# erick093/MPI_Pytorch

Hardware: AMD Instinct MI355X
Metric: images/sec (whole node) ResNet-18 224x224 training at 1/2/4/8 MI355X (higher is better)
Workload: dtype bf16; 1 GPU; model=resnet18, global_batch=2048, per_gpu_batch=2048, image_size=224, num_classes=64500, optimizer=adam, parallelism=dp1, device=cuda, backend=none, hip_graph=False, deterministic=True

## Files before the change

### csrc/bindings.cpp

```cpp
#include <torch/extension.h>
#include <c10/hip/HIPStream.h>
#include <c10/core/DeviceGuard.h>

#include <vector>

#include "kernels/api.h"
#include "runtime/runtime.h"

using torch::Tensor;

namespace {

inline hipStream_t cur_stream() { return c10::hip::getCurrentHIPStream().stream(); }

#define CHECK_CUDA(x) TORCH_CHECK((x).is_cuda(), #x " must be a GPU tensor")
#define CHECK_CONTIG(x) TORCH_CHECK((x).is_contiguous(), #x " must be contiguous")
#define CHECK_BF16(x) \
  TORCH_CHECK((x).scalar_type() == torch::kBFloat16, #x " must be bfloat16, got ", (x).scalar_type())
#define CHECK_F32(x) \
  TORCH_CHECK((x).scalar_type() == torch::kFloat32, #x " must be float32, got ", (x).scalar_type())
#define CHECK_ACT(x) \
  CHECK_CUDA(x);     \
  CHECK_CONTIG(x);   \
  CHECK_BF16(x)
// ... 425 lines not shown

void bn_defer_step(Tensor sums, Tensor gamma, Tensor mean, Tensor rstd, int64_t s0, Tensor k12,
                   Tensor dgamma, Tensor dbeta, Tensor G, Tensor x, c10::optional<Tensor> out) {
  CHECK_CUDA(G);
  CHECK_CONTIG(G);
  CHECK_ACT(x);
  CHECK_F32(k12);
  CHECK_CONTIG(k12);
  const int Ci = sums.numel() / 2;
  const int ctot = x.size(-1);
  const int M = x.numel() / ctot;
  TORCH_CHECK(x.is_contiguous() && G.sizes() == x.sizes() && k12.numel() == 2 * ctot,
              "bn_defer_step: G / x / k12 shapes");
  TORCH_CHECK(s0 >= 0 && s0 < Ci && Ci <= ctot && (Ci - s0) % 8 == 0 &&
                  256 % ((Ci - s0) / 8) == 0,
              "bn_defer_step: slice [s0, Ci) must be 8-channel groups dividing 256");
  for (const Tensor* t : {&gamma, &mean, &rstd}) {
    CHECK_F32(*t);
    TORCH_CHECK(t->numel() >= Ci, "bn_defer_step: per-channel vector size");
  }
  const bool into = out && out->defined() && out->numel() > 0;
  if (into) {
    CHECK_ACT((*out));
    TORCH_CHECK(out->is_contiguous() && out->size(-1) == Ci - s0 && out->numel() / (Ci - s0) == M,
                "bn_defer_step: out must be a contiguous bf16 [..., Ci - s0]");
  }
  const c10::OptionalDeviceGuard g(device_of(x));
  mpa::bn_defer_step(sums.data_ptr<float>(), gamma.data_ptr<float>(), mean.data_ptr<float>(),
                     rstd.data_ptr<float>(), Ci, (int)s0, M, k12.data_ptr<float>(), ctot,
                     fopt_mut(dgamma), fopt_mut(dbeta), G.data_ptr(),
                     G.scalar_type() == torch::kFloat32, ctot, bp(x), ctot,
                     into ? bpm(*out) : nullptr, cur_stream());
}

static int row_stride(const Tensor& t);

std::vector<Tensor> bn_bwd_apply(Tensor dy, Tensor x, Tensor y, Tensor mean, Tensor rstd,
                                 Tensor gamma, Tensor dgamma, Tensor dbeta, Tensor sums,
                                 bool want_dx, bool want_g) {
  CHECK_CUDA(dy);
  CHECK_BF16(dy);
  const int lddy = row_stride(dy);
  CHECK_ACT(x);
  const int C = x.size(-1);
  const int M = x.numel() / C;
  TORCH_CHECK(C % 8 == 0 && sums.numel() == 2 * C && dy.size(-1) == C && lddy % 8 == 0,
              "bn_bwd_apply: shapes");
  TORCH_CHECK(aligned16(dy),
              "bn_bwd_apply: dy must start on a 16-byte boundary (channel offset % 8 == 0)");
  const c10::OptionalDeviceGuard g(device_of(x));
  Tensor dx = want_dx ? torch::empty_like(x) : Tensor();
  Tensor gout = want_g ? torch::empty_like(x) : Tensor();
  mpa::bn_bwd_apply(bp(dy), bp(x), bopt(y), fopt(mean), fopt(rstd), fopt(gamma),
                    fopt_mut(dgamma), fopt_mut(dbeta), M, C, want_dx ? bpm(dx) : nullptr,
                    want_g ? bpm(gout) : nullptr, fopt(sums), cur_stream(), lddy);
  return {dx, gout};
}

void conv_wgrad(Tensor dy, Tensor x, Tensor dw, int64_t sh, int64_t sw, int64_t ph, int64_t pw,
                bool overwrite) {
  CHECK_ACT(dy);
  CHECK_ACT(x);
  CHECK_CUDA(dw);
  CHECK_F32(dw);
  CHECK_CONTIG(dw);
  const int N = x.size(0), H = x.size(1), W = x.size(2), C = x.size(3);
  const int P = dy.size(1), Q = dy.size(2), K = dy.size(3);
  TORCH_CHECK(dw.dim() == 4 && dw.size(0) == K && dw.size(3) == C, "conv_wgrad: dw shape");
  const int R = dw.size(1), S = dw.size(2);
  TORCH_CHECK(dy.size(0) == N, "conv_wgrad: batch mismatch");
  const c10::OptionalDeviceGuard g(device_of(dy));
  mpa::WGradArgs a{};
  a.dy = bp(dy); a.x = bp(x); a.dw = dw.data_ptr<float>();
  a.Kout = K; a.C = C; a.H = H; a.W = W; a.P = P; a.Q = Q; a.R = R; a.S = S;
  a.sh = sh; a.sw = sw; a.ph = ph; a.pw = pw;
  a.Mpix = N * P * Q;
  a.Ncols = R * S * C;
  a.overwrite = overwrite ? 1 : 0;
  Tensor slab;
  a.slab = alloc_ws(slab, dy, mpa::igemm_wgrad_ws_floats(a.Kout, a.Ncols, a.Mpix));
  mpa::igemm_wgrad(a, vec_width(K), (C % 8 == 0) ? 8 : 1, cur_stream());
}

Tensor act_bwd(Tensor dy, Tensor y, Tensor dbias) {
  CHECK_ACT(dy);
  const int C = dy.size(-1);
  const int M = dy.numel() / C;
  const bool hy = has(y);
  if (!hy && !has(dbias)) return dy;
  const c10::OptionalDeviceGuard g(device_of(dy));
  Tensor out = hy ? torch::empty_like(dy) : dy;
  Tensor ws;
  float* wsp = nullptr;
  if (has(dbias) && C % 8 == 0) {
    ws = torch::empty({mpa::bn_ws_floats(M, C)}, dy.options().dtype(torch::kFloat32));
    wsp = ws.data_ptr<float>();
  }
  mpa::act_bwd(bp(dy), hy ? bopt(y) : nullptr, fopt_mut(dbias), M, C, hy ? bpm(out) : nullptr,
               wsp, cur_stream());
  return out;
}

static uint8_t* ymask_ptr(const c10::optional<Tensor>& m, const Tensor& like) {
  if (!m || !m->defined() || m->numel() == 0) return nullptr;
  TORCH_CHECK(m->scalar_type() == torch::kUInt8 && m->is_contiguous() && m->numel() == like.numel() / 8 &&
                  m->device() == like.device(),
              "bn: ReLU mask must be contiguous uint8 [numel / 8] on the activation's device");
  return m->data_ptr<uint8_t>();
}

static int row_stride(const Tensor& t) {
  TORCH_CHECK(t.dim() >= 1 && t.stride(-1) == 1, "bn: channels must be contiguous");
  if (t.dim() == 1) return (int)t.size(0);
  const int64_t ld = t.stride(-2);
  int64_t expect = ld * t.size(-2);
  for (int64_t d = t.dim() - 3; d >= 0; --d) {
    TORCH_CHECK(t.size(d) == 1 || t.stride(d) == expect, "bn: rows must be uniformly strided");
    expect *= t.size(d);
  }
  TORCH_CHECK(ld >= t.size(-1), "channel window: row stride below the row width");
  return (int)ld;
}

static void bn_prefix(const Tensor& x, int64_t channels, int* C, int* ldx, int* M) {
  CHECK_CUDA(x);
  CHECK_BF16(x);
  if (channels > 0) {
    CHECK_CONTIG(x);
    *ldx = x.size(-1);
    *C = (int)channels;
  } else {
    *ldx = row_stride(x);
    *C = x.size(-1);
  }
  TORCH_CHECK(*C <= *ldx && *C % 8 == 0 && *ldx % 8 == 0,
              "bn: channels must be a multiple of 8 within the row");
  TORCH_CHECK(aligned16(x), "bn: x must start on a 16-byte boundary (channel offset % 8 == 0)");
  *M = x.numel() / x.size(-1);
}

static std::vector<int64_t> with_last(const Tensor& x, int64_t c) {
  std::vector<int64_t> shape(x.sizes().begin(), x.sizes().end());
  shape.back() = c;
  return shape;
}

std::vector<Tensor> bn_fwd_train(Tensor x, Tensor stats, Tensor gamma, Tensor beta, Tensor rmean,
                                 Tensor rvar, double momentum, double eps, Tensor res, bool relu,
                                 c10::optional<Tensor> counter, c10::optional<Tensor> mask,
                                 int64_t channels, c10::optional<Tensor> res_affine,
                                 c10::optional<Tensor> out) {
  int C, ldx, M;
  bn_prefix(x, channels, &C, &ldx, &M);
  const c10::OptionalDeviceGuard g(device_of(x));
  const bool into = out && out->defined() && out->numel() > 0;
  int ldy = C;
  if (into) {
    CHECK_CUDA(*out);
    CHECK_BF16(*out);
    TORCH_CHECK(out->sizes() == c10::IntArrayRef(with_last(x, C)) && !has(res) &&
                    !(mask && mask->defined() && mask->numel()),
                "bn_fwd_train: out must have the output's shape (no residual / mask)");
    ldy = row_stride(*out);
    TORCH_CHECK(ldy % 8 == 0, "bn_fwd_train: out row stride must be a multiple of 8");
    TORCH_CHECK(aligned16(*out),
                "bn_fwd_train: out must start on a 16-byte boundary (channel offset % 8 == 0)");
// ... 1153 lines not shown
  CHECK_CUDA(g);
  CHECK_CONTIG(g);
  CHECK_F32(g);
  const int64_t ctot = g.size(-1);
  TORCH_CHECK(ctot % 8 == 0 && cs % 8 == 0 && off % 8 == 0 && off >= 0 && off + cs <= ctot && cs > 0,
              "chan_extract: channel range outside G (multiples of 8 required)");
  const int64_t pixels = g.numel() / ctot;
  TORCH_CHECK(pixels * (cs / 8) < (int64_t(1) << 31), "chan_extract: too large");
  const c10::OptionalDeviceGuard gd(device_of(g));
  std::vector<int64_t> shape(g.sizes().begin(), g.sizes().end());
  shape.back() = cs;
  Tensor out = torch::empty(shape, g.options().dtype(torch::kBFloat16));
  if (pixels > 0)
    mpa::chan_extract(g.data_ptr<float>(), (int)ctot, (int)off, bpm(out), (int)cs, (int)pixels,
                      cur_stream());
  return out;
}

std::vector<Tensor> split_channels(Tensor dy, std::vector<int64_t> sizes) {
  CHECK_ACT(dy);
  TORCH_CHECK(dy.dim() >= 2 && !sizes.empty(), "split_channels: dy must be [..., C]");
  int64_t ctot = 0;
  for (int64_t c : sizes) {
    TORCH_CHECK(c > 0 && c % 8 == 0, "split_channels: channels must be a multiple of 8");
    ctot += c;
  }
  TORCH_CHECK(ctot == dy.size(-1), "split_channels: sizes do not sum to C");
  const int64_t pixels = dy.numel() / ctot;
  TORCH_CHECK(pixels * (ctot / 8) < (int64_t(1) << 31), "split_channels: too large");
  const c10::OptionalDeviceGuard g(device_of(dy));
  std::vector<Tensor> out;
  std::vector<mpa::bf16_raw*> ptrs;
  std::vector<int> chans;
  std::vector<int64_t> shape(dy.sizes().begin(), dy.sizes().end());
  for (int64_t c : sizes) {
    shape.back() = c;
    out.push_back(torch::empty(shape, dy.options()));
    ptrs.push_back(bpm(out.back()));
    chans.push_back((int)c);
  }
  if (pixels > 0)
    mpa::split_channels(bp(dy), chans.data(), (int)sizes.size(), (int)pixels, (int)ctot,
                        ptrs.data(), cur_stream());
  return out;
}

}

extern "C" const char* mpa_src_hash();

PYBIND11_MODULE(TORCH_EXTENSION_NAME, m) {
  m.doc() = "mpi_pytorch_amd native gfx950 kernels + runtime";
  m.def("src_hash", [] { return std::string(mpa_src_hash()); },
        "hash of the csrc/ sources this binary was built from (setup.py source_hash)");
  m.def("igemm_engine", &mpa::igemm_engine, "GEMM staging engine: 1 LDS-DMA, 0 register");
  m.def("igemm_set_engine", &mpa::igemm_set_engine);
  m.def("igemm_force_tile", &mpa::igemm_force_tile, "override GEMM tile (BM, BN, splits); 0 = auto");
  m.def("igemm_set_tune", &mpa::igemm_set_tune, "tile autotuner on/off (MPA_TUNE)");
  m.def("igemm_set_tune_drain", &mpa::igemm_set_tune_drain,
        "tuner candidates: drain the whole device (1, single GPU) or only their stream (0)");
  m.def("set_deterministic", &mpa::set_deterministic,
        "fixed-order reductions + no timing-based autotuning (MPA_DETERMINISTIC)");
  m.def("deterministic", &mpa::deterministic);
  m.def("igemm_tuned_table", &mpa::igemm_tuned_table, "autotuned GEMM tiles so far");
  m.def("igemm_tuned_load", &mpa::igemm_tuned_load, py::arg("table"), py::arg("replace") = true,
        "adopt an igemm_tuned_table() dump (data-parallel ranks take rank 0's)");
  m.def("igemm_set_dma_uni", &mpa::igemm_set_dma_uni, "LDS-DMA uniform-tap fast path on/off");
  m.def("igemm_set_halo", &mpa::igemm_set_halo, "halo-staged direct 3x3/s1 conv on/off");
  m.def("igemm_set_halo_mi7", &mpa::igemm_set_halo_mi7, "448-pixel halo tiles on/off");
  m.def("igemm_set_halo_strip", &mpa::igemm_set_halo_strip,
        "strip-tiled halo conv: 0 off, 1 images too wide for linear tiles, 2 also layer1");
  m.def("igemm_halo_enabled", &mpa::igemm_halo_enabled);
  m.def("igemm_set_stem", &mpa::igemm_set_stem, "direct row-staged 7x7 pixel-pair stem on/off");
  m.def("preprocess_set_copy", &mpa::preprocess_set_copy,
        "identity-size preprocess fast path on/off (MPA_PRE_COPY)");
  m.def("set_comm_reserve", &mpa::set_comm_reserve,
        "CUs held by an overlapping collective (persistent conv grids use the rest)");
  m.def("comm_reserve", &mpa::comm_reserve, "current collective CU reservation");
  m.def("active_cus", &mpa::active_cus, "CUs the persistent conv grids size for");
  m.def("igemm_set_halo_wprod", &mpa::igemm_set_halo_wprod,
        "halo weight gradients on producer-wave blocks on/off (MPA_HALO_WPROD)");
  m.def("igemm_set_halo_wxmap", &mpa::igemm_set_halo_wxmap,
        "XCD-grouped halo weight-gradient block order on/off (MPA_HALO_WXMAP)");
  m.def("affine_act", &affine_act, "relu?(x * aff[0] + aff[1]) per channel (aff [2, C])");
  m.def("conv_fwd", &conv_fwd, py::arg("x"), py::arg("w"), py::arg("bias"), py::arg("sh"),
        py::arg("sw"), py::arg("ph"), py::arg("pw"), py::arg("relu"), py::arg("stats"),
        py::arg("shift"), "conv forward (+ BN statistics of its output)");
  m.def("conv_dgrad", &conv_dgrad, py::arg("dy"), py::arg("w"), py::arg("H"), py::arg("W"),
        py::arg("sh"), py::arg("sw"), py::arg("ph"), py::arg("pw"), py::arg("wt") = py::none(),
        py::arg("accum") = py::none());
  m.def("conv_wgrad", &conv_wgrad, py::arg("dy"), py::arg("x"), py::arg("dw"), py::arg("sh"),
        py::arg("sw"), py::arg("ph"), py::arg("pw"), py::arg("overwrite") = false,
        "weight gradient into dw (+=; overwrite: dw = ..., the first gradient since zero)");
  m.def("conv_bnred_ok", &conv_bnred_ok);
  m.def("conv_dgrad_bnred_gacc", &conv_dgrad_bnred_gacc);
  m.def("conv_dgrad_res", &conv_dgrad_res);
  m.def("conv_dgrad_pair", &conv_dgrad_pair, py::arg("dy"), py::arg("w"), py::arg("wt"),
        py::arg("H"), py::arg("W"), py::arg("sh"), py::arg("sw"), py::arg("ph"), py::arg("pw"),
        py::arg("dy2"), py::arg("w2"), py::arg("wt2"), py::arg("ph2"), py::arg("pw2"),
        py::arg("accum") = py::none());
  m.def("bn_defer_step", &bn_defer_step, py::arg("sums"), py::arg("gamma"), py::arg("mean"),
        py::arg("rstd"), py::arg("s0"), py::arg("k12"), py::arg("dgamma"), py::arg("dbeta"),
        py::arg("G"), py::arg("x"), py::arg("out") = py::none());
  m.def("conv_fwd_into", &conv_fwd_into);
  m.def("conv_dgrad_bnred", &conv_dgrad_bnred, py::arg("dy"), py::arg("w"), py::arg("H"),
        py::arg("W"), py::arg("sh"), py::arg("sw"), py::arg("ph"), py::arg("pw"), py::arg("wt"),
        py::arg("z"), py::arg("y"), py::arg("mean"), py::arg("rstd"),
        py::arg("gamma") = py::none(), py::arg("beta") = py::none());
  m.def("bn_bwd_apply", &bn_bwd_apply);
  m.def("act_bwd", &act_bwd);
  m.def("bn_fwd_train", &bn_fwd_train, py::arg("x"), py::arg("stats"), py::arg("gamma"),
        py::arg("beta"), py::arg("rmean"), py::arg("rvar"), py::arg("momentum"), py::arg("eps"),
        py::arg("res"), py::arg("relu"), py::arg("counter") = py::none(),
        py::arg("mask") = py::none(), py::arg("channels") = 0,
        py::arg("res_affine") = py::none(), py::arg("out") = py::none());
  m.def("bn_stats_affine", &bn_stats_affine, py::arg("x"), py::arg("stats"), py::arg("gamma"),
        py::arg("beta"), py::arg("rmean"), py::arg("rvar"), py::arg("momentum"),
        py::arg("eps"), py::arg("counter") = py::none());
  m.def("bn_stats", &bn_stats, "[mean | biased var] of x [..., C]");
  m.def("bn_relu_avgpool2_fwd", &bn_relu_avgpool2_fwd);
  m.def("bn_fwd_eval", &bn_fwd_eval, py::arg("x"), py::arg("gamma"), py::arg("beta"),
        py::arg("rmean"), py::arg("rvar"), py::arg("eps"), py::arg("res"), py::arg("relu"),
        py::arg("channels") = 0);
  m.def("bn_bwd_pair", &bn_bwd_pair);
  m.def("maxpool_bwd_relu", &maxpool_bwd_relu);
  m.def("bn_bwd", &bn_bwd, py::arg("dy"), py::arg("x"), py::arg("y"), py::arg("mean"),
        py::arg("rstd"), py::arg("gamma"), py::arg("dgamma"), py::arg("dbeta"),
        py::arg("want_dx"), py::arg("want_g"), py::arg("zmask_beta") = py::none(),
        py::arg("ymask") = py::none(), py::arg("gacc") = py::none(),
        py::arg("dx_out") = py::none());
  m.def("relu_fwd", &relu_fwd);
  m.def("comm_emulator", &comm_emulator, "diagnostics: occupy CUs like a concurrent collective");
  m.def("atomic_latency", &atomic_latency, "diagnostics: dependent atomic round trips");
  m.def("maxpool_fwd", &maxpool_fwd);
  m.def("maxpool_bwd", &maxpool_bwd);
  m.def("bn_relu_maxpool_fwd", &bn_relu_maxpool_fwd, py::arg("z"), py::arg("stats"),
        py::arg("gamma"), py::arg("beta"), py::arg("rmean"), py::arg("rvar"), py::arg("momentum"),
        py::arg("eps"), py::arg("kh"), py::arg("kw"), py::arg("sh"), py::arg("sw"), py::arg("ph"),
        py::arg("pw"), py::arg("ceil"), py::arg("counter") = py::none(),
        py::arg("zsel_out") = py::none());
  m.def("maxpool_bn_bwd_sums", &maxpool_bn_bwd_sums);
  m.def("stem_pool_wgrad_ok", &stem_pool_wgrad_ok);
  m.def("stem_pool_wgrad", &stem_pool_wgrad);
  m.def("maxpool_bn_bwd", &maxpool_bn_bwd, py::arg("dp"), py::arg("idx"), py::arg("z"),
        py::arg("mean"), py::arg("rstd"), py::arg("gamma"), py::arg("beta"), py::arg("dgamma"),
        py::arg("dbeta"), py::arg("kh"), py::arg("kw"), py::arg("sh"), py::arg("sw"),
        py::arg("ph"), py::arg("pw"), py::arg("zsel") = py::none());
  m.def("avgpool_fwd", &avgpool_fwd);
  m.def("avgpool_bwd", &avgpool_bwd, py::arg("dy"), py::arg("H"), py::arg("W"), py::arg("kh"),
        py::arg("kw"), py::arg("sh"), py::arg("sw"), py::arg("ph"), py::arg("pw"),
        py::arg("ceil"), py::arg("cip"), py::arg("dx_out") = py::none());
  m.def("adaptive_avgpool_fwd", &adaptive_avgpool_fwd);
  m.def("adaptive_avgpool_bwd", &adaptive_avgpool_bwd);
  m.def("linear_fwd", &linear_fwd);
  m.def("linear_dgrad", &linear_dgrad, py::arg("dy"), py::arg("w"), py::arg("wt") = py::none());
  m.def("linear_wgrad", &linear_wgrad, py::arg("dy"), py::arg("x"), py::arg("dw"),
        py::arg("overwrite") = false);
  m.def("ce_fwd", &ce_fwd, py::arg("logits"), py::arg("labels"), py::arg("smoothing") = 0.0,
        py::arg("labels2") = py::none(), py::arg("lam") = py::none());
  m.def("ce_bwd", &ce_bwd, py::arg("logits"), py::arg("labels"), py::arg("lse"),
        py::arg("grad_out"), py::arg("weight") = 1.0, py::arg("smoothing") = 0.0,
        py::arg("labels2") = py::none(), py::arg("lam") = py::none());
  m.def("ce_fwd_weighted", &ce_fwd_weighted, py::arg("logits"), py::arg("labels"),
        py::arg("out"), py::arg("acc"), py::arg("weight"), py::arg("accumulate"),
        py::arg("smoothing") = 0.0, py::arg("labels2") = py::none(), py::arg("lam") = py::none());
  m.def("argmax_correct", &argmax_correct);
// ... 43 lines not shown
```

### csrc/kernels/api.h

```cpp
#pragma once
#include <algorithm>
#include <string>
#include <hip/hip_runtime.h>
#include <stdint.h>

namespace mpa {

typedef uint16_t bf16_raw;
constexpr int MAXT = 128;

struct Taps {
  short dh[MAXT];
  short dw[MAXT];
  short bt[MAXT];
};

struct FastDiv {
  uint32_t m, s;
};
inline FastDiv make_fastdiv(uint32_t d) {
  if (d <= 1) return FastDiv{0u, 0u};
  const uint32_t l = 32u - (uint32_t)__builtin_clz(d - 1u);
  return FastDiv{(uint32_t)(((1ull << (31 + l)) + d - 1) / d), l - 1u};
}
// ... 40 lines not shown
  const float* ep_gamma;
  const float* ep_beta;
  void* ep_gacc;
  int ep_gacc_f32;
  int stap;
  int beta;
  FastDiv fd_hw, fd_ow;
  const bf16_raw* A2;
  const bf16_raw* B2;
  int ldb2;
  int kpad;
  const bf16_raw* ep_res;
  const uint8_t* ep_rmask;
};
constexpr short TAP_SRC2 = 0x2000;

inline void igemm_set_fastdiv(IGemmArgs& a) {
  a.fd_hw = make_fastdiv((uint32_t)std::max(1, a.oH * a.oW));
  a.fd_ow = make_fastdiv((uint32_t)std::max(1, a.oW));
  for (int i = 0; i < a.nphase && i < MAXPH; ++i) {
    a.ph[i].fd_hw = make_fastdiv((uint32_t)std::max(1, a.ph[i].oH * a.ph[i].oW));
    a.ph[i].fd_ow = make_fastdiv((uint32_t)std::max(1, a.ph[i].oW));
  }
}

struct WGradArgs {
  const bf16_raw* dy;
  const bf16_raw* x;
  float* dw;
  float* slab;
  int Kout, C, H, W, P, Q, R, S, sh, sw, ph, pw;
  int Mpix;
  int Ncols;
  int ktiles_per_split;
  int tiles_n, tiles_total;
  int overwrite;
};

int64_t igemm_slab_floats(int M, int N);
void igemm_rows(IGemmArgs a, int vw, float* ws, float* slab, hipStream_t s);
void igemm_rows_dgrad(IGemmArgs a, int vw, float* ws, hipStream_t s, bool bkc = false);
void igemm_rows_dgrad_phases(IGemmArgs a, int vw, hipStream_t s, bool bkc = false);
bool igemm_dgrad_src2_ok(const IGemmArgs& a, int vw, bool bkc);
int64_t igemm_bnred_slab_floats(int M, int N, int nphase);
void igemm_rows_dgrad_bnred(IGemmArgs a, int vw, bool bkc, float* slab, float* sums,
                            hipStream_t s);
void igemm_wgrad(WGradArgs a, int vwa, int vwb, hipStream_t s);
int64_t igemm_ws_floats(int M, int N, int Ktot);
int64_t igemm_wgrad_ws_floats(int Kout, int Ncols, int Mpix);
int igemm_engine();
void igemm_set_engine(int engine);
void igemm_force_tile(int bm, int bn, int splits);
void igemm_set_tune(int on);
void igemm_set_tune_drain(int on);
std::string igemm_tuned_table();
int igemm_tuned_load(const std::string& table, bool replace);
void igemm_set_dma_uni(int on);
bool igemm_stap_ok();
bool conv3_halo_ok(const IGemmArgs& a);
int conv3_halo(IGemmArgs a, hipStream_t s);
constexpr int HALO_MAX_ROWS = 256;
void igemm_set_halo(int on);
void igemm_set_halo_mi7(int on);
void igemm_set_halo_strip(int mode);
bool stem_wgrad_ok(const WGradArgs& a);
int stem_wgrad(WGradArgs a, hipStream_t s);
int64_t stem_wgrad_ws_floats();
struct StemPoolArgs {
  const bf16_raw* dp;
  const uint8_t* idx;
  const float *mean, *rstd, *gamma, *beta;
  const float* sums;
  int PP, PQ;
  float invM;
};
bool stem_pool_wgrad_ok(const WGradArgs& a, const StemPoolArgs& q);
int stem_pool_wgrad(WGradArgs a, StemPoolArgs q, hipStream_t s);
void igemm_stem_pool_wgrad(WGradArgs a, StemPoolArgs q, hipStream_t s);
bool conv3_halo_wgrad_ok(const WGradArgs& a);
void igemm_set_halo_wxmap(int on);
void igemm_set_halo_wprod(int on);
int conv3_halo_wgrad(WGradArgs a, hipStream_t s);
int64_t conv3_halo_wgrad_ws_floats(int Kout, int Ncols);
bool igemm_halo_enabled();
void set_comm_reserve(int cus);
int comm_reserve();
int active_cus();
bool conv_stem_ok(const IGemmArgs& a);
int conv_stem(IGemmArgs a, hipStream_t s);
void igemm_set_stem(int on);

int64_t bn_ws_floats(int M, int C);
void slab_reduce(const float* slab, int S, int W, float* out, bool zero_out, hipStream_t s);
bool dense_gacc_ok(const IGemmArgs& a);
void dense_gacc(IGemmArgs a, float* slab, float* sums, hipStream_t s);
void bn_defer_step(const float* sums, const float* gamma, const float* mean, const float* rstd,
                   int Ci, int s0, int M, float* k12, int ldk, float* dgamma, float* dbeta,
                   void* G, bool g_f32, int ldg, const bf16_raw* x, int ldx, bf16_raw* out,
                   hipStream_t s);
void set_deterministic(int on);
bool deterministic();
void slab_stats(float* slab, int S, int C, const float* shift, int M, float* sums, float* out,
                hipStream_t s, int out_ld = 0);
void stats_finalize(const float* sums, const float* shift, int M, int C, float* out,
                    hipStream_t s);
void bn_stats(const bf16_raw* x, int M, int C, const float* shift, float* stats, float* ws,
              hipStream_t s);
void bn_fwd_train(const bf16_raw* x, const float* stats, const float* gamma, const float* beta,
                  float* rmean, float* rvar, float momentum, float eps, const bf16_raw* res,
                  int relu, int M, int C, bf16_raw* y, float* mean, float* rstd,
                  int64_t* counter, hipStream_t s,
                  uint8_t* ymask = nullptr,
                  int ldx = 0,
                  int lds = 0,
                  const float* res_aff = nullptr,
                  int ldy = 0);
void bn_stats_affine(const float* stats, const float* gamma, const float* beta, float* rmean,
                     float* rvar, float momentum, float eps, int M, int C, float* mean,
                     float* rstd, float* aff, int64_t* counter, hipStream_t s);
void bn_relu_avgpool2_fwd(const bf16_raw* z, const float* aff, int N, int H, int W, int C,
                          bf16_raw* y, hipStream_t s);
void affine_act(const bf16_raw* x, const float* aff, int relu, int M, int C, bf16_raw* y,
                hipStream_t s);
void bn_fwd_eval(const bf16_raw* x, const float* gamma, const float* beta, const float* rmean,
                 const float* rvar, float eps, const bf16_raw* res, int relu, int M, int C,
                 bf16_raw* y, hipStream_t s, int ldx = 0);
void bn_bwd(const bf16_raw* dy, const bf16_raw* x, const bf16_raw* y, const float* mean,
            const float* rstd, const float* gamma, float* dgamma, float* dbeta, int M, int C,
            bf16_raw* dx, bf16_raw* g, float* ws, hipStream_t s,
            const float* zmask_beta = nullptr,
            const uint8_t* ymask = nullptr,
            int ldx = 0,
            float* gacc = nullptr,
            int ldg = 0,
            int lddx = 0,
            bool gacc_bf16 = false,
            int lddy = 0);
bool maxpool2_ok(int N, int H, int W, int C, int kh, int kw, int sh, int sw, int ph, int pw);
void maxpool2_fwd(const bf16_raw* x, int N, int H, int W, int C, bf16_raw* y, uint8_t* idx,
                  hipStream_t s);
int64_t maxpool2_ws_floats(int N, int H, int W, int C);
void maxpool2_bwd(const bf16_raw* dy, const uint8_t* idx, const bf16_raw* yp, int N, int H, int W,
                  int C, bf16_raw* dx, float* sums, float* ws, hipStream_t s);
int64_t bn_pair_ws_floats(int M, int C);
void bn_bwd_pair(const bf16_raw* dy, const bf16_raw* x, const bf16_raw* x2, const uint8_t* ymask,
                 const float* mean, const float* rstd, const float* gamma, const float* mean2,
                 const float* rstd2, const float* gamma2, float* dgamma, float* dbeta,
                 float* dgamma2, float* dbeta2, int M, int C, bf16_raw* dx, bf16_raw* dx2,
                 float* ws, hipStream_t s);
void bn_bwd_apply(const bf16_raw* dy, const bf16_raw* x, const bf16_raw* y, const float* mean,
                  const float* rstd, const float* gamma, float* dgamma, float* dbeta, int M,
                  int C, bf16_raw* dx, bf16_raw* g, const float* sums, hipStream_t s,
                  int lddy = 0);
void act_bwd(const bf16_raw* dy, const bf16_raw* y, float* dbias, int M, int C, bf16_raw* g,
             float* ws, hipStream_t s);
void relu_fwd(const bf16_raw* x, int64_t n, bf16_raw* y, hipStream_t s);
void bn_relu_maxpool_fwd(const bf16_raw* z, const float* stats, const float* gamma,
                         const float* beta, float* rmean, float* rvar, float momentum, float eps,
                         int N, int H, int W, int C, int P, int Q, int kh, int kw, int sh, int sw,
                         int ph, int pw, bf16_raw* y, uint8_t* idx, float* mean, float* rstd,
                         int64_t* counter, hipStream_t s, bf16_raw* zsel = nullptr);
int64_t maxpool_bn_ws_floats(int M, int C);
void maxpool_bn_bwd_sums(const bf16_raw* dp, const bf16_raw* zsel, const float* mean,
                         const float* rstd, const float* gamma, const float* beta, float* dgamma,
                         float* dbeta, int MP, int C, float* ws, hipStream_t s);
void maxpool_bn_bwd(const bf16_raw* dp, const uint8_t* idx, const bf16_raw* z, const float* mean,
// ... 140 lines not shown
```

### csrc/kernels/conv_halo.hip

```cpp
#include <algorithm>
#include <atomic>
#include <cstdlib>
#include <type_traits>
#include "igemm_common.h"

namespace mpa {

constexpr int HB_BM = 256, HB_BN = 64, HB_NW = 4;
constexpr int HB_HIW = 9;
constexpr int HB_HPX = 16 * HB_NW * HB_HIW;
constexpr int HB_HBYTES = HB_HPX * 64;
constexpr int HB_WIW = 9;
constexpr int HB_WBYTES = 9 * HB_BN * 64;
constexpr int HB_RED = HB_NW * HB_BN * 2 * 4;
constexpr int HB_COLS = 4 * HB_BN * 4;
constexpr int HB_LDS = 2 * HB_HBYTES + 2 * HB_WBYTES + HB_RED + HB_COLS;

struct HaloPlan {
  int w2;
  int btoff[9];
  uint32_t mag_w, mag_w2, mag_h1, mag_hw;
  int tiles_m, tiles_total, cc;
  uint32_t a_bytes, b_bytes;
};

__device__ __forceinline__ bf16x8 frag16(const char* lds_byte) {
  return __builtin_bit_cast(bf16x8, *LDS_PTR(const u32x4, lds_byte));
}

enum : int { EP_RELU = 1, EP_BETA = 2, EP_BNRED = 4, EP_STATS = 8, EP_BIAS = 16 };

template <int MI = 4>
struct EpiInT {
  uint2 a[MI][4];
  uint2 mk[MI];
};
typedef EpiInT<4> EpiIn;

__device__ __forceinline__ uint2 acc_operand(const IGemmArgs& p, uint32_t e) {
  return *(const uint2*)((const bf16_t*)(p.ep_res ? p.ep_res : p.C) + e);
}

__device__ __forceinline__ uint2 acc_mask(const IGemmArgs& p, uint32_t e0) {
  return p.ep_rmask ? *(const uint2*)(p.ep_rmask + (e0 >> 3)) : make_uint2(~0u, ~0u);
}

__device__ __forceinline__ uint2 masked_acc(uint2 v, uint2 mk, int jn, int jq) {
  const uint32_t word = jn < 2 ? mk.x : mk.y;
  const uint32_t nib = (word >> ((16 * jn + 4 * jq) & 31)) & 15u;
  v.x &= ((nib & 1u) ? 0xffffu : 0u) | ((nib & 2u) ? 0xffff0000u : 0u);
  v.y &= ((nib & 4u) ? 0xffffu : 0u) | ((nib & 8u) ? 0xffff0000u : 0u);
  return v;
}

template <int EPI, int NJ, int MI = 4>
__device__ __forceinline__ void epi_preload(const IGemmArgs& p, EpiInT<MI>& in, int m0, int n0,
                                            int wave, int lane) {
  if constexpr (!(EPI & (EP_BETA | EP_BNRED))) {
#pragma unroll
    for (int i = 0; i < MI; ++i)
#pragma unroll
      for (int jn = 0; jn < 4; ++jn) in.a[i][jn] = make_uint2(0u, 0u);
  } else {
    const int nl = (lane >> 4) * 4;
#pragma unroll
    for (int i = 0; i < MI; ++i) {
      const int m = min(m0 + wave * 16 * MI + i * 16 + (lane & 15), p.M - 1);
      const uint32_t orow = (uint32_t)m * p.ldc + n0 + nl;
      if constexpr (!(EPI & EP_BNRED)) in.mk[i] = acc_mask(p, (uint32_t)m * p.ldc + n0);
#pragma unroll
      for (int jn = 0; jn < NJ; ++jn) {
        if constexpr (EPI & EP_BNRED) {
          in.a[i][jn] = *(const uint2*)(p.ep_z + orow + jn * 16);
        } else {
          in.a[i][jn] = acc_operand(p, orow + jn * 16);
        }
      }
    }
  }
}

__device__ __forceinline__ float lo_f(uint32_t w) { return __uint_as_float(w << 16); }
__device__ __forceinline__ float hi_f(uint32_t w) { return __uint_as_float(w & 0xffff0000u); }

template <int EPI, bool FULL, bool ST = true>
// ... 838 lines not shown
  const int wave_all = __builtin_amdgcn_readfirstlane(tid >> 6);
  const int wave = wave_all & 3;
  const int H = p.H, W = p.W, HW = H * W, W2 = W2T ? W2T : h.w2, C = p.C, K = p.Kout;
  const int M = p.Mpix, nimg = M / HW;
  const int g = lane >> 4, li = lane & 15, q = li >> 2, pp = li & 3;

  const int bid = h.xmap ? (blockIdx.x & 7) * (gridDim.x >> 3) + (blockIdx.x >> 3) : blockIdx.x;
  const int part = bid % h.parts, z = bid / h.parts;
  const int k0 = (part % h.kparts) * 64, c0 = (part / h.kparts) * 64;
  const int ntiles = z < h.tiles_m ? (h.tiles_m - z + h.Z - 1) / h.Z : 0;

  uint32_t drow[4];
  bool kok[4];
#pragma unroll
  for (int j = 0; j < 4; ++j) {
    const int row = 8 * (4 * wave + j) + (lane >> 3);
    const int chunk = (lane & 7) ^ mn_swz<64>(row & 31);
    drow[j] = ((uint32_t)(STRIP ? 0 : row) * K + k0 + chunk * 8) * 2;
    kok[j] = k0 + chunk * 8 < K;
  }
  uint32_t hsc[HIW];
#pragma unroll
  for (int j = 0; j < HIW; ++j) {
    const uint32_t hp = 16 * (wave * HIW + j) + (lane >> 2);
    const uint32_t sl = udiv(hp, h.mag_w2);
    const uint32_t colp = hp - sl * W2;
    const uint32_t lc = (lane & 3) ^ (((hp >> 3) & 1) << 1);
    hsc[j] = sl | (colp << 10) | (lc << 18);
  }
  const __amdgpu_buffer_rsrc_t rdy = make_rsrc(p.dy, h.dy_bytes);
  const __amdgpu_buffer_rsrc_t rx0 = make_rsrc(p.x, h.x_bytes);
  const __amdgpu_buffer_rsrc_t rx1 =
      make_rsrc((const char*)p.x + 64, c0 + 32 < C ? h.x_bytes : 0u);
  uint32_t hv[HIW], dv[4];
  const int cbyte = ((2 * (wave & 1) + (pp >> 1)) << 4) + 8 * (pp & 1);
  const int hoff = HW_DBYTES + (ONECH ? 0 : (wave >> 1) * HW_HBYTES);
  auto stage_base = [&](int st) { return st * HW_STAGE + hoff - W2 * 64; };
  int hbw[4][2][3];
  const int tpx = STRIP ? h.tr * h.tw : HW_BM;
  if constexpr (STRIP) {
#pragma unroll
    for (int ks = 0; ks < 4; ++ks)
#pragma unroll
      for (int e = 0; e < 2; ++e) {
        const uint32_t n = (uint32_t)min(ks * 32 + 8 * g + 4 * e + q, tpx - 1);
        const uint32_t lr = udiv1(n, h.mag_tw), lc = n - lr * h.tw;
        const int hp = (int)(lr + 1) * W2 + (int)lc + 1;
#pragma unroll
        for (int d = 0; d < 3; ++d) {
          const int x = (hp + d - 1) * 64 + cbyte;
          hbw[ks][e][d] = (x ^ ((x >> 4) & 32)) + stage_base(0);
        }
      }
  }
  auto prep_dma = [&](int mt) {
    if constexpr (STRIP) {
      const int img = (int)udiv1((uint32_t)mt, h.mag_timg);
      const uint32_t rem = (uint32_t)(mt - img * h.tiles_img);
      const uint32_t band = udiv1(rem, h.mag_tc);
      const int r0 = (int)band * h.tr, cs0 = (int)(rem - band * h.tiles_c) * h.tw;
#pragma unroll
      for (int j = 0; j < HIW; ++j) {
        const int sl = hsc[j] & 1023, col = (int)((hsc[j] >> 10) & 255);
        const int ih = r0 - p.ph + sl, iw = cs0 - p.pw + col;
        const bool ok = sl < h.tr + 2 && col < h.tw + 2 && (unsigned)ih < (unsigned)H &&
                        (unsigned)iw < (unsigned)W;
        hv[j] = ok ? ((((uint32_t)img * H + ih) * W + iw) * C + c0) * 2 + (hsc[j] >> 18) * 16
                   : 0x80000000u;
      }
#pragma unroll
      for (int j = 0; j < 4; ++j) {
        const uint32_t row = 8 * (4 * wave + j) + (lane >> 3);
        const uint32_t lr = udiv1(row, h.mag_tw), lc = row - lr * h.tw;
        const bool ok = (int)row < tpx && r0 + (int)lr < p.P && cs0 + (int)lc < p.Q && kok[j];
        dv[j] = ok ? drow[j] + (((uint32_t)img * p.P + r0 + lr) * p.Q + cs0 + lc) * (uint32_t)K * 2
                   : 0x80000000u;
      }
      return;
    }
    const int m0 = mt * HW_BM;
    const int img0 = m0 / HW;
    const int r0 = m0 - img0 * HW;
    const int oh0 = r0 / W;
#pragma unroll
    for (int j = 0; j < HIW; ++j) {
      const int sl = hsc[j] & 1023, col = (int)((hsc[j] >> 10) & 255) - 1;
      const int v = sl + oh0 - 1;
      const int d = (int)udiv((uint32_t)(v + H + 1), h.mag_h1) - 1;
      const int row = v - d * (H + 1);
      const int img = img0 + d;
      const bool ok = row < H && (unsigned)col < (unsigned)W && img < nimg;
      hv[j] = ok ? ((((uint32_t)img * H + row) * W + col) * C + c0) * 2 + (hsc[j] >> 18) * 16
                 : 0x80000000u;
    }
#pragma unroll
    for (int j = 0; j < 4; ++j) {
      const int row = 8 * (4 * wave + j) + (lane >> 3);
      dv[j] = (m0 + row < M && kok[j]) ? drow[j] + (uint32_t)m0 * K * 2 : 0x80000000u;
    }
  };
  auto prep_b = [&](int mt, int st) {
    if constexpr (STRIP) {
      const int dlt = st ? HW_STAGE : -HW_STAGE;
#pragma unroll
      for (int ks = 0; ks < 4; ++ks)
#pragma unroll
        for (int e = 0; e < 2; ++e)
#pragma unroll
          for (int d = 0; d < 3; ++d) hbw[ks][e][d] += dlt;
    } else {
      const int hb0 = stage_base(st);
      const int m0 = mt * HW_BM;
      const int img0 = m0 / HW;
      const int r0 = m0 - img0 * HW;
      const int oh0 = r0 / W;
      const int mlast = M - 1 - img0 * HW;
#pragma unroll
      for (int ks = 0; ks < 4; ++ks)
#pragma unroll
        for (int e = 0; e < 2; ++e) {
          const uint32_t n = (uint32_t)min(r0 + ks * 32 + 8 * g + 4 * e + q, mlast);
          const uint32_t di = udiv(n, h.mag_hw);
          const uint32_t rem = n - di * HW;
          const uint32_t oh = udiv(rem, h.mag_w);
          const uint32_t ow = rem - oh * W;
          const int hp = ((int)(di * (H + 1) + oh) - oh0 + 1) * W2 + (int)ow + 1;
#pragma unroll
          for (int d = 0; d < 3; ++d) {
            const int x = (hp + d - 1) * 64 + cbyte;
            hbw[ks][e][d] = (x ^ ((x >> 4) & 32)) + hb0;
          }
        }
    }
  };
  const uint32_t sw = lds_base(smem) + wave * 4096;
  auto dmaw = [&](int stage, int j) {
    const uint32_t st = sw + stage * HW_STAGE;
    if (j < 4) {
      buf_lds16_at(rdy, st + j * 1024, dv[j]);
    } else if constexpr (ONECH) {
      const int jj = j - 4;
      buf_lds16_at(rx0, st - wave * 4096 + HW_DBYTES + (wave * HIW + jj) * 1024, hv[jj]);
    } else {
      const int ch = (j - 4) / HW_HIW, jj = (j - 4) % HW_HIW;
      buf_lds16_at(ch ? rx1 : rx0, st - wave * 4096 + HW_DBYTES + ch * HW_HBYTES +
                                       (wave * HW_HIW + jj) * 1024, hv[jj]);
    }
  };
  auto issue = [&](int stage) {
#pragma unroll
    for (int j = 0; j < 4 + 2 * HW_HIW; ++j) dmaw(stage, j);
  };

  if constexpr (PROD) {
    if (wave_all >= 4) {
      if (ntiles > 0) {
        prep_dma(z);
        issue(0);
      }
      for (int k = 0; k < ntiles; ++k) {
        asm volatile("s_waitcnt vmcnt(0)" ::: "memory");
        __builtin_amdgcn_s_barrier();
        if (k + 1 < ntiles) {
          prep_dma(z + (k + 1) * h.Z);
          issue((k + 1) & 1);
        }
      }
      return;
    }
  }

  f32x4 acc[KM][9];
#pragma unroll
  for (int km = 0; km < KM; ++km)
// ... 331 lines not shown
}

static int g_halo_mi7 = [] {
  const char* e = getenv("MPA_HALO_MI7");
  return e ? atoi(e) : 1;
}();
void igemm_set_halo_mi7(int on) { g_halo_mi7 = on; }

static bool halo_mi7_ok(const IGemmArgs& a, int epi, bool wres) {
  if (!g_halo_mi7 || !wres || a.N != HB_BN) return false;
  if (epi != 0 && epi != EP_STATS) return false;
  int ch, cw;
  if (!tap_shift(a, ch, cw) || ch != 0 || cw != 0) return false;
  const int64_t HW = (int64_t)a.aH * a.aW;
  constexpr int BM7 = 448;
  if (HW % BM7 != 0 || BM7 % a.aW != 0 || a.M % BM7 != 0) return false;
  return (BM7 / a.aW + 2) * halo_pitch(a.aW) <= 640;
}

template <int EPI>
static void launch_halo32(bool wres, int grid, const IGemmArgs& a, const HaloPlan& h,
                          hipStream_t s) {
  launch_halo_k<EPI, 2>(wres, grid, a, h, s);
}

int conv3_halo(IGemmArgs a, hipStream_t s) {
  {
    bool linear;
    halo_ok_impl(a, linear);
    if (use_strip(a, linear)) return conv3_strip(a, s);
  }
  HaloPlan h{};
  const int W2 = halo_pitch(a.aW);
  h.w2 = W2;
  for (int t = 0; t < 9; ++t) {
    const int r = (a.Oh + a.taps.dh[t] + 1) * 3 + (a.Ow + a.taps.dw[t] + 1);
    h.btoff[r] = a.taps.bt[t] * a.aC * 2;
  }
  h.mag_w = magic(a.aW);
  h.mag_w2 = magic(W2);
  h.mag_h1 = magic(a.aH + 1);
  h.mag_hw = magic(a.aH * a.aW);
  h.cc = a.aC / 32;
  const bool wres = g_halo_wres && (a.N + HB_BN - 1) / HB_BN == 1 && h.cc <= 2;
  const bool mi7 = halo_mi7_ok(a, halo_epi(a), wres);
  h.tiles_m = mi7 ? a.M / 448 : (a.M + HB_BM - 1) / HB_BM;
  a.tiles_n = (a.N + HB_BN - 1) / HB_BN;
  h.tiles_total = h.tiles_m * a.tiles_n;
  a.tiles_total = h.tiles_total;
  h.a_bytes = (uint32_t)((int64_t)a.M * a.aC * 2);
  h.b_bytes = (uint32_t)((int64_t)a.N * a.ldb * 2);
  int g8 = std::min(std::min(active_cus(), HALO_MAX_ROWS) / 8, (h.tiles_total + 7) / 8);
  g8 = std::max(a.tiles_n, g8 / a.tiles_n * a.tiles_n);
  const int grid = 8 * g8;
  if (a.N == 32) {
    if (halo_epi(a) == EP_STATS) launch_halo32<EP_STATS>(wres, grid, a, h, s);
    else launch_halo32<0>(wres, grid, a, h, s);
    return grid;
  }
  switch (halo_epi(a)) {
    case 0: launch_halo<0>(wres, grid, a, h, s, mi7); break;
    case EP_BETA: launch_halo<EP_BETA>(wres, grid, a, h, s); break;
    case EP_STATS: launch_halo<EP_STATS>(wres, grid, a, h, s, mi7); break;
    case EP_BIAS | EP_RELU: launch_halo<EP_BIAS | EP_RELU>(wres, grid, a, h, s); break;
    case EP_BIAS | EP_STATS: launch_halo<EP_BIAS | EP_STATS>(wres, grid, a, h, s); break;
    default: launch_halo<EP_BNRED>(wres, grid, a, h, s); break;
  }
  return grid;
}

static int halo_wgrad_pitch(int W) { return (W + 2 + 15) / 16 * 16; }

static bool halo_wgrad_base(const WGradArgs& a) {
  if (!g_halo || a.R != 3 || a.S != 3 || a.sh != 1 || a.sw != 1) return false;
  if (a.ph < 0 || a.ph > 1 || a.pw < 0 || a.pw > 1) return false;
  if (a.P != a.H + 2 * a.ph - 2 || a.Q != a.W + 2 * a.pw - 2 || a.P <= 0 || a.Q <= 0) return false;
  if (a.C % 32 != 0 || a.Kout % 32 != 0) return false;
  const int64_t PQ = (int64_t)a.P * a.Q;
  if (a.Mpix % PQ != 0) return false;
  const int64_t nimg = a.Mpix / PQ;
  return nimg * a.H * a.W * a.C * 2 < (1ll << 31) && (int64_t)a.Mpix * a.Kout * 2 < (1ll << 31);
}

static bool halo_wgrad_strip_plan(const WGradArgs& a, HaloWPlan& h) {
  if (g_strip < 1 || !halo_wgrad_base(a)) return false;
  const int OH = a.P, OW = a.Q;
  const int64_t nimg = a.Mpix / ((int64_t)OH * OW);
  int64_t best = -1;
  for (int n = 1; n <= OW; ++n) {
    const int tw = (OW + n - 1) / n;
    if (tw > 126 || (n > 1 && (OW + tw - 1) / tw != n)) continue;
    if (tw < 8) break;
    const int pitch = (tw + 2 + 15) / 16 * 16;
    int tr = std::max(1, std::min(OH, HW_BM / tw));
    while (tr > 1 && (tr + 2) * pitch > HW_HPX) --tr;
    if ((tr + 2) * pitch > HW_HPX) continue;
    const int64_t tiles = nimg * ((OH + tr - 1) / tr) * n;
    const int64_t cost = tiles * (HW_BM + (tr + 2) * pitch);
    if (best < 0 || cost < best) {
      best = cost;
      h.tr = tr;
      h.tw = tw;
      h.w2 = pitch;
      h.tiles_c = n;
      h.tiles_img = ((OH + tr - 1) / tr) * n;
      h.tiles_m = (int)tiles;
    }
  }
  if (best < 0 || h.tiles_m <= 0) return false;
  h.mag_tw = magic(h.tw);
  h.mag_tc = h.tiles_c > 1 ? magic(h.tiles_c) : 0u;
  h.mag_timg = h.tiles_img > 1 ? magic(h.tiles_img) : 0u;
  return true;
}

static bool halo_wgrad_geom(const WGradArgs& a) {
  if (!halo_wgrad_base(a) || a.ph != 1 || a.pw != 1) return false;
  const int64_t HW = (int64_t)a.H * a.W;
  if (HW + HW_BM >= 65536 || a.W + 2 > 255) return false;
  const int64_t rows = (HW_BM - 1 + a.W - 1) / a.W + 1;
  const int64_t seps = (HW_BM - 1) / HW + 1;
  return (rows + 2 + seps) * halo_wgrad_pitch(a.W) <= (a.C == 32 ? 2 : 1) * HW_HPX;
}

static bool halo_wgrad_onech(const WGradArgs& a) {
  const int64_t HW = (int64_t)a.H * a.W;
  const int64_t rows = (HW_BM - 1 + a.W - 1) / a.W + 1;
  const int64_t seps = (HW_BM - 1) / HW + 1;
  return a.C == 32 && (rows + 2 + seps) * halo_wgrad_pitch(a.W) > HW_HPX;
}

int64_t conv3_halo_wgrad_ws_floats(int Kout, int Ncols) {
  if (Ncols % 9 != 0 || (Ncols / 9) % 32 != 0 || Kout % 32 != 0) return 0;
  return (int64_t)HALO_MAX_ROWS * 64 * 64 * 9;
}

bool conv3_halo_wgrad_ok(const WGradArgs& a) {
  if (a.slab == nullptr) return false;
  if (halo_wgrad_geom(a)) return true;
  HaloWPlan h{};
  return halo_wgrad_strip_plan(a, h);
}

static bool g_wxmap = [] {
  const char* e = getenv("MPA_HALO_WXMAP");
  return !(e && e[0] == '0');
}();

static bool g_wprod = [] {
  const char* e = getenv("MPA_HALO_WPROD");
  return !(e && e[0] == '0');
}();
void igemm_set_halo_wprod(int on) { g_wprod = on != 0; }
void igemm_set_halo_wxmap(int on) { g_wxmap = on != 0; }

template <int W2T, bool ONECH = false, bool STRIP = false>
static void launch_halo_wgrad(const WGradArgs& a, const HaloWPlan& h, dim3 grid, hipStream_t s) {
  if constexpr (!STRIP) {
    if (g_wprod) {
      if (a.Kout == 32)
        hipLaunchKernelGGL((conv3_halo_wgrad_kernel<0, ONECH, false, true, 2>), grid,
                           dim3(512), 0, s, a, h);
      else
        hipLaunchKernelGGL((conv3_halo_wgrad_kernel<0, ONECH, false, true>), grid,
                           dim3(512), 0, s, a, h);
      return;
    }
  }
  hipLaunchKernelGGL((conv3_halo_wgrad_kernel<W2T, ONECH, STRIP>), grid, dim3(256), 0, s, a, h);
}

int conv3_halo_wgrad(WGradArgs a, hipStream_t s) {
  HaloWPlan h{};
  if (!halo_wgrad_geom(a) && halo_wgrad_strip_plan(a, h)) {
    const int W2 = h.w2;
    for (int t = 0; t < 9; ++t) h.toff[t] = (t / 3 - 1) * W2 + (t % 3 - 1);
    h.mag_w2 = magic(W2);
    h.kparts = (a.Kout + 63) / 64;
    h.parts = h.kparts * ((a.C + 63) / 64);
    const int G = std::min(active_cus(), HALO_MAX_ROWS);
    h.Z = std::max(1, std::min(G / h.parts, h.tiles_m));
    h.dy_bytes = (uint32_t)((int64_t)a.Mpix * a.Kout * 2);
    h.x_bytes = (uint32_t)((int64_t)(a.Mpix / ((int64_t)a.P * a.Q)) * a.H * a.W * a.C * 2);
    h.xmap = g_wxmap && (h.parts * h.Z) % 8 == 0;
    launch_halo_wgrad<0, false, true>(a, h, dim3(h.parts * h.Z), s);
    return h.Z;
  }
  const int W2 = halo_wgrad_pitch(a.W);
  h.w2 = W2;
  for (int t = 0; t < 9; ++t) h.toff[t] = (t / 3 - 1) * W2 + (t % 3 - 1);
  h.mag_w = magic(a.W);
  h.mag_w2 = magic(W2);
  h.mag_h1 = magic(a.H + 1);
  h.mag_hw = magic(a.H * a.W);
  h.tiles_m = (a.Mpix + HW_BM - 1) / HW_BM;
  h.kparts = (a.Kout + 63) / 64;
  h.parts = h.kparts * ((a.C + 63) / 64);
  const int G = std::min(active_cus(), HALO_MAX_ROWS);
  h.Z = std::max(1, std::min(G / h.parts, h.tiles_m));
  h.dy_bytes = (uint32_t)((int64_t)a.Mpix * a.Kout * 2);
  h.x_bytes = (uint32_t)((int64_t)a.Mpix * a.C * 2);
  const dim3 grid(h.parts * h.Z);
  h.xmap = g_wxmap && (h.parts * h.Z) % 8 == 0;
  if (halo_wgrad_onech(a)) {
    launch_halo_wgrad<0, true>(a, h, grid, s);
    return h.Z;
  }
  switch (W2) {
    case 16: launch_halo_wgrad<16>(a, h, grid, s); break;
    case 32: launch_halo_wgrad<32>(a, h, grid, s); break;
    case 48: launch_halo_wgrad<48>(a, h, grid, s); break;
    case 64: launch_halo_wgrad<64>(a, h, grid, s); break;
    default: launch_halo_wgrad<0>(a, h, grid, s); break;
  }
  return h.Z;
}

}
```

Before: 55880 images/sec.

## Choose halo weight-gradient tiling by a byte/row cost model between linear and strips

Adds a cost model that compares the halo-loaded input pixels and GEMM rows of linear tiles against 2D strip tiles. Strips are chosen automatically when they move markedly fewer bytes without too many extra rows, and the choice is cached per shape. Strip tiling now prefers row counts that divide the output height, and can run on producer-wave 512-thread blocks or a pitch-16 specialisation. Linear tiles also skip halo rows past the tile's last pixel. The exchange is more host-side planning and new kernel instantiations, with the risk that strips lose efficiency on some shapes.

```diff
diff --git a/csrc/bindings.cpp b/csrc/bindings.cpp
--- a/csrc/bindings.cpp
+++ b/csrc/bindings.cpp
@@ -531,6 +531,22 @@
   mpa::igemm_wgrad(a, vec_width(K), (C % 8 == 0) ? 8 : 1, cur_stream());
 }
 
+py::dict halo_wgrad_tiles(int64_t N, int64_t H, int64_t W, int64_t C, int64_t K, int64_t pad) {
+  mpa::WGradArgs a{};
+  a.Kout = K; a.C = C; a.H = H; a.W = W; a.P = H + 2 * pad - 2; a.Q = W + 2 * pad - 2;
+  a.R = 3; a.S = 3; a.sh = 1; a.sw = 1; a.ph = pad; a.pw = pad;
+  a.Mpix = N * a.P * a.Q;
+  a.Ncols = 9 * C;
+  const mpa::HaloWTiles t = mpa::conv3_halo_wgrad_tiles(a);
+  py::dict d;
+  d["tiling"] = t.tiling; d["tr"] = t.tr; d["tw"] = t.tw;
+  d["lin_x_px"] = t.lin_x_px; d["lin_dy_px"] = t.lin_dy_px; d["lin_rows"] = t.lin_rows;
+  d["lin_bytes"] = t.lin_bytes;
+  d["strip_x_px"] = t.strip_x_px; d["strip_dy_px"] = t.strip_dy_px;
+  d["strip_rows"] = t.strip_rows; d["strip_bytes"] = t.strip_bytes;
+  return d;
+}
+
 Tensor act_bwd(Tensor dy, Tensor y, Tensor dbias) {
   CHECK_ACT(dy);
   const int C = dy.size(-1);
@@ -1850,6 +1866,11 @@
         "halo weight gradients on producer-wave blocks on/off (MPA_HALO_WPROD)");
   m.def("igemm_set_halo_wxmap", &mpa::igemm_set_halo_wxmap,
         "XCD-grouped halo weight-gradient block order on/off (MPA_HALO_WXMAP)");
+  m.def("igemm_set_halo_wgrad_tiles", &mpa::igemm_set_halo_wgrad_tiles,
+        "halo weight-gradient tiling: 0 byte model, 1 linear, 2 strips (MPA_HALO_WTILES)");
+  m.def("halo_wgrad_tiles", &halo_wgrad_tiles, py::arg("N"), py::arg("H"), py::arg("W"),
+        py::arg("C"), py::arg("K"), py::arg("pad") = 1,
+        "tiling the halo weight gradient takes for a shape, and its byte model");
   m.def("affine_act", &affine_act, "relu?(x * aff[0] + aff[1]) per channel (aff [2, C])");
   m.def("conv_fwd", &conv_fwd, py::arg("x"), py::arg("w"), py::arg("bias"), py::arg("sh"),
         py::arg("sw"), py::arg("ph"), py::arg("pw"), py::arg("relu"), py::arg("stats"),
diff --git a/csrc/kernels/api.h b/csrc/kernels/api.h
--- a/csrc/kernels/api.h
+++ b/csrc/kernels/api.h
@@ -146,6 +146,14 @@
 void igemm_set_halo_wprod(int on);
 int conv3_halo_wgrad(WGradArgs a, hipStream_t s);
 int64_t conv3_halo_wgrad_ws_floats(int Kout, int Ncols);
+void igemm_set_halo_wgrad_tiles(int mode);
+struct HaloWTiles {
+  int tiling;
+  int tr, tw;
+  int64_t lin_x_px, lin_dy_px, lin_rows, lin_bytes;
+  int64_t strip_x_px, strip_dy_px, strip_rows, strip_bytes;
+};
+HaloWTiles conv3_halo_wgrad_tiles(const WGradArgs& a);
 bool igemm_halo_enabled();
 void set_comm_reserve(int cus);
 int comm_reserve();
diff --git a/csrc/kernels/conv_halo.hip b/csrc/kernels/conv_halo.hip
--- a/csrc/kernels/conv_halo.hip
+++ b/csrc/kernels/conv_halo.hip
@@ -1,6 +1,9 @@
 #include <algorithm>
+#include <array>
 #include <atomic>
 #include <cstdlib>
+#include <map>
+#include <mutex>
 #include <type_traits>
 #include "igemm_common.h"
 
@@ -1005,6 +1008,9 @@
     const int img0 = m0 / HW;
     const int r0 = m0 - img0 * HW;
     const int oh0 = r0 / W;
+    const uint32_t last = (uint32_t)min(r0 + HW_BM - 1, M - 1 - img0 * HW);
+    const uint32_t dl = udiv(last, h.mag_hw);
+    const int nsl = (int)(dl * (H + 1) + udiv(last - dl * HW, h.mag_w)) - oh0 + 3;
 #pragma unroll
     for (int j = 0; j < HIW; ++j) {
       const int sl = hsc[j] & 1023, col = (int)((hsc[j] >> 10) & 255) - 1;
@@ -1012,7 +1018,7 @@
       const int d = (int)udiv((uint32_t)(v + H + 1), h.mag_h1) - 1;
       const int row = v - d * (H + 1);
       const int img = img0 + d;
-      const bool ok = row < H && (unsigned)col < (unsigned)W && img < nimg;
+      const bool ok = sl < nsl && row < H && (unsigned)col < (unsigned)W && img < nimg;
       hv[j] = ok ? ((((uint32_t)img * H + row) * W + col) * C + c0) * 2 + (hsc[j] >> 18) * 16
                  : 0x80000000u;
     }
@@ -1510,32 +1516,61 @@
   return nimg * a.H * a.W * a.C * 2 < (1ll << 31) && (int64_t)a.Mpix * a.Kout * 2 < (1ll << 31);
 }
 
+struct HaloWCost {
+  int64_t x_px, dy_px, rows;
+};
+
+static int64_t halo_wgrad_bytes(const WGradArgs& a, const HaloWCost& c) {
+  const int64_t kparts = (a.Kout + 63) / 64, cparts = (a.C + 63) / 64;
+  return c.dy_px * a.Kout * 2 * cparts + c.x_px * a.C * 2 * kparts;
+}
+
+static int64_t halo_window_sum(int out, int t, int pad, int in) {
+  int64_t sum = 0;
+  for (int t0 = 0; t0 < out; t0 += t)
+    sum += std::min(in, t0 - pad + t + 2) - std::max(0, t0 - pad);
+  return sum;
+}
+
+static HaloWCost halo_wgrad_strip_cost(const WGradArgs& a, int tr, int tw) {
+  const int64_t nimg = a.Mpix / ((int64_t)a.P * a.Q);
+  HaloWCost c;
+  c.x_px = nimg * halo_window_sum(a.P, tr, a.ph, a.H) * halo_window_sum(a.Q, tw, a.pw, a.W);
+  c.dy_px = a.Mpix;
+  c.rows = nimg * ((a.P + tr - 1) / tr) * ((a.Q + tw - 1) / tw) * HW_BM;
+  return c;
+}
+
 static bool halo_wgrad_strip_plan(const WGradArgs& a, HaloWPlan& h) {
   if (g_strip < 1 || !halo_wgrad_base(a)) return false;
   const int OH = a.P, OW = a.Q;
   const int64_t nimg = a.Mpix / ((int64_t)OH * OW);
-  int64_t best = -1;
+  int64_t best_px = -1, best_rows = 0;
   for (int n = 1; n <= OW; ++n) {
     const int tw = (OW + n - 1) / n;
     if (tw > 126 || (n > 1 && (OW + tw - 1) / tw != n)) continue;
     if (tw < 8) break;
     const int pitch = (tw + 2 + 15) / 16 * 16;
-    int tr = std::max(1, std::min(OH, HW_BM / tw));
-    while (tr > 1 && (tr + 2) * pitch > HW_HPX) --tr;
-    if ((tr + 2) * pitch > HW_HPX) continue;
-    const int64_t tiles = nimg * ((OH + tr - 1) / tr) * n;
-    const int64_t cost = tiles * (HW_BM + (tr + 2) * pitch);
-    if (best < 0 || cost < best) {
-      best = cost;
+    int trmax = std::max(1, std::min(OH, HW_BM / tw));
+    while (trmax > 1 && (trmax + 2) * pitch > HW_HPX) --trmax;
+    if ((trmax + 2) * pitch > HW_HPX) continue;
+    int trdiv = trmax;
+    while (OH % trdiv != 0) --trdiv;
+    for (int tr : {trdiv, trmax}) {
+      const HaloWCost c = halo_wgrad_strip_cost(a, tr, tw);
+      if (best_px >= 0 && (c.x_px > best_px || (c.x_px == best_px && c.rows >= best_rows)))
+        continue;
+      best_px = c.x_px;
+      best_rows = c.rows;
       h.tr = tr;
       h.tw = tw;
       h.w2 = pitch;
       h.tiles_c = n;
       h.tiles_img = ((OH + tr - 1) / tr) * n;
-      h.tiles_m = (int)tiles;
-    }
-  }
-  if (best < 0 || h.tiles_m <= 0) return false;
+      h.tiles_m = (int)(nimg * h.tiles_img);
+    }
+  }
+  if (best_px < 0 || h.tiles_m <= 0) return false;
   h.mag_tw = magic(h.tw);
   h.mag_tc = h.tiles_c > 1 ? magic(h.tiles_c) : 0u;
   h.mag_timg = h.tiles_img > 1 ? magic(h.tiles_img) : 0u;
@@ -1558,6 +1593,76 @@
   return a.C == 32 && (rows + 2 + seps) * halo_wgrad_pitch(a.W) > HW_HPX;
 }
 
+static HaloWCost halo_wgrad_linear_cost(const WGradArgs& a) {
+  const int H = a.H, W = a.W, HW = H * W, M = a.Mpix, nimg = M / HW;
+  const int slots = (halo_wgrad_onech(a) ? 2 : 1) * HW_HPX / halo_wgrad_pitch(W);
+  const int tiles = (M + HW_BM - 1) / HW_BM;
+  HaloWCost c{0, M, (int64_t)tiles * HW_BM};
+  for (int mt = 0; mt < tiles; ++mt) {
+    const int m0 = mt * HW_BM, img0 = m0 / HW, r0 = m0 - img0 * HW, oh0 = r0 / W;
+    const int last = std::min(r0 + HW_BM - 1, M - 1 - img0 * HW);
+    const int nsl = std::min(slots, (last / HW) * (H + 1) + (last % HW) / W - oh0 + 3);
+    for (int sl = oh0 ? 0 : 1; sl < nsl; ++sl) {
+      const int v = sl + oh0 - 1, d = v / (H + 1);
+      if (v - d * (H + 1) < H && img0 + d < nimg) c.x_px += W;
+    }
+  }
+  return c;
+}
+
+static int g_wtiles = [] {
+  const char* e = getenv("MPA_HALO_WTILES");
+  return e ? atoi(e) : 0;
+}();
+void igemm_set_halo_wgrad_tiles(int mode) { g_wtiles = mode; }
+
+constexpr int WT_BYTES = 80, WT_ROWS = 120;
+
+static bool halo_wgrad_auto_strips(const WGradArgs& a, const HaloWPlan& h) {
+  if (a.C % 64 != 0 || a.Kout % 64 != 0) return false;
+  static std::mutex mu;
+  static std::map<std::array<int, 5>, bool> seen;
+  const std::array<int, 5> key{a.H, a.W, a.C, a.Kout, a.Mpix};
+  std::lock_guard<std::mutex> lock(mu);
+  auto it = seen.find(key);
+  if (it != seen.end()) return it->second;
+  const HaloWCost lin = halo_wgrad_linear_cost(a), st = halo_wgrad_strip_cost(a, h.tr, h.tw);
+  const bool strips = halo_wgrad_bytes(a, st) * 100 <= halo_wgrad_bytes(a, lin) * WT_BYTES &&
+                      st.rows * 100 <= lin.rows * WT_ROWS;
+  seen[key] = strips;
+  return strips;
+}
+
+static int halo_wgrad_choice(const WGradArgs& a, HaloWPlan& h) {
+  const bool lin = halo_wgrad_geom(a), strip = halo_wgrad_strip_plan(a, h);
+  if (!lin || !strip) return lin ? 1 : strip ? 2 : 0;
+  if (g_wtiles == 1 || g_wtiles == 2) return g_wtiles;
+  return halo_wgrad_auto_strips(a, h) ? 2 : 1;
+}
+
+HaloWTiles conv3_halo_wgrad_tiles(const WGradArgs& a) {
+  HaloWTiles t{};
+  HaloWPlan h{};
+  t.tiling = halo_wgrad_choice(a, h);
+  if (halo_wgrad_geom(a)) {
+    const HaloWCost c = halo_wgrad_linear_cost(a);
+    t.lin_x_px = c.x_px;
+    t.lin_dy_px = c.dy_px;
+    t.lin_rows = c.rows;
+    t.lin_bytes = halo_wgrad_bytes(a, c);
+  }
+  if (halo_wgrad_strip_plan(a, h)) {
+    const HaloWCost c = halo_wgrad_strip_cost(a, h.tr, h.tw);
+    t.tr = h.tr;
+    t.tw = h.tw;
+    t.strip_x_px = c.x_px;
+    t.strip_dy_px = c.dy_px;
+    t.strip_rows = c.rows;
+    t.strip_bytes = halo_wgrad_bytes(a, c);
+  }
+  return t;
+}
+
 int64_t conv3_halo_wgrad_ws_floats(int Kout, int Ncols) {
   if (Ncols % 9 != 0 || (Ncols / 9) % 32 != 0 || Kout % 32 != 0) return 0;
   return (int64_t)HALO_MAX_ROWS * 64 * 64 * 9;
@@ -1583,8 +1688,15 @@
 void igemm_set_halo_wxmap(int on) { g_wxmap = on != 0; }
 
 template <int W2T, bool ONECH = false, bool STRIP = false>
-static void launch_halo_wgrad(const WGradArgs& a, const HaloWPlan& h, dim3 grid, hipStream_t s) {
-  if constexpr (!STRIP) {
+static void launch_halo_wgrad(const WGradArgs& a, const HaloWPlan& h, dim3 grid, hipStream_t s,
+                              bool prod = true) {
+  if constexpr (STRIP) {
+    if (g_wprod && prod) {
+      hipLaunchKernelGGL((conv3_halo_wgrad_kernel<0, false, true, true>), grid, dim3(512), 0, s,
+                         a, h);
+      return;
+    }
+  } else {
     if (g_wprod) {
       if (a.Kout == 32)
         hipLaunchKernelGGL((conv3_halo_wgrad_kernel<0, ONECH, false, true, 2>), grid,
@@ -1600,7 +1712,8 @@
 
 int conv3_halo_wgrad(WGradArgs a, hipStream_t s) {
   HaloWPlan h{};
-  if (!halo_wgrad_geom(a) && halo_wgrad_strip_plan(a, h)) {
+  if (halo_wgrad_choice(a, h) == 2) {
+    const bool lin = halo_wgrad_geom(a);
     const int W2 = h.w2;
     for (int t = 0; t < 9; ++t) h.toff[t] = (t / 3 - 1) * W2 + (t % 3 - 1);
     h.mag_w2 = magic(W2);
@@ -1611,9 +1724,11 @@
     h.dy_bytes = (uint32_t)((int64_t)a.Mpix * a.Kout * 2);
     h.x_bytes = (uint32_t)((int64_t)(a.Mpix / ((int64_t)a.P * a.Q)) * a.H * a.W * a.C * 2);
     h.xmap = g_wxmap && (h.parts * h.Z) % 8 == 0;
-    launch_halo_wgrad<0, false, true>(a, h, dim3(h.parts * h.Z), s);
+    if (W2 == 16) launch_halo_wgrad<16, false, true>(a, h, dim3(h.parts * h.Z), s, lin);
+    else launch_halo_wgrad<0, false, true>(a, h, dim3(h.parts * h.Z), s, lin);
     return h.Z;
   }
+  h = HaloWPlan{};
   const int W2 = halo_wgrad_pitch(a.W);
   h.w2 = W2;
   for (int t = 0; t < 9; ++t) h.toff[t] = (t / 3 - 1) * W2 + (t % 3 - 1);
```

Measured after the change: 56400 images/sec, median of 6. About the same (+0.9%).
